# humeniuka/semiclassical

Measured on AMD Instinct MI355X. Metric: trajectory-steps/sec + wall-time to converged C(t), anharmonic-AS D=60, higher is better.
Workload: dtype f64

## Files before the change

### semiclassical_amd/csrc/sc_hk_lu.h

```cpp
#pragma once
#include "sc_common.h"

#ifdef LU_PIVOT_CLOCK
static __device__ unsigned long long *g_lu_clock = nullptr;
#endif

namespace {

template <int CTRL>
__device__ __forceinline__ int dpp_mov_i32(int v) {
    return __builtin_amdgcn_update_dpp(v, v, CTRL, 0xF, 0xF, false);
}

__device__ __forceinline__ int row16_max_i32(int v) {
    asm("s_nop 1\n\t"
        "v_max_i32_dpp %0, %0, %0 row_ror:8 row_mask:0xf bank_mask:0xf\n\ts_nop 1\n\t"
        "v_max_i32_dpp %0, %0, %0 row_ror:4 row_mask:0xf bank_mask:0xf\n\ts_nop 1\n\t"
        "v_max_i32_dpp %0, %0, %0 row_ror:2 row_mask:0xf bank_mask:0xf\n\ts_nop 1\n\t"
        "v_max_i32_dpp %0, %0, %0 row_ror:1 row_mask:0xf bank_mask:0xf"
        : "+v"(v));
    return v;
}

__device__ __forceinline__ double readlane_f64(double v, int src) {
    const int lo = __builtin_amdgcn_readlane(__double2loint(v), src);
    const int hi = __builtin_amdgcn_readlane(__double2hiint(v), src);
    return __hiloint2double(hi, lo);
}

__device__ __forceinline__ cplx c_inv_fast(cplx z) {
    const double x = c_abs2(z);
    double r = __builtin_amdgcn_rcp(x);
    r = fma(fma(-x, r, 1.0), r, r);
    r = fma(fma(-x, r, 1.0), r, r);
    return c_make(z.x * r, -z.y * r);
}

struct PivotRecord {
    int col, pad;
};

#define SC_DPP_MOV(o, i, P) "v_mov_b64_dpp %[" #o "], %[" #i "] row_newbcast:" #P " row_mask:0xf bank_mask:0xf\n\t"
#define SC_LEAF1(P) SC_DPP_MOV(ox0, ix0, P) SC_DPP_MOV(oy0, iy0, P) "s_branch .Lend_%=\n\t"
#define SC_LEAF2(P) SC_DPP_MOV(ox0, ix0, P) SC_DPP_MOV(oy0, iy0, P) SC_DPP_MOV(ox1, ix1, P) SC_DPP_MOV(oy1, iy1, P) \
    "s_branch .Lend_%=\n\t"
#define SC_LEAF3(P) SC_DPP_MOV(ox0, ix0, P) SC_DPP_MOV(oy0, iy0, P) SC_DPP_MOV(ox1, ix1, P) SC_DPP_MOV(oy1, iy1, P) \
    SC_DPP_MOV(ox2, ix2, P) SC_DPP_MOV(oy2, iy2, P) "s_branch .Lend_%=\n\t"
#define SC_LEAF4(P) SC_DPP_MOV(ox0, ix0, P) SC_DPP_MOV(oy0, iy0, P) SC_DPP_MOV(ox1, ix1, P) SC_DPP_MOV(oy1, iy1, P) \
    SC_DPP_MOV(ox2, ix2, P) SC_DPP_MOV(oy2, iy2, P) SC_DPP_MOV(ox3, ix3, P) SC_DPP_MOV(oy3, iy3, P) "s_branch .Lend_%=\n\t"
#define SC_LEAF5(P) SC_DPP_MOV(ox0, ix0, P) SC_DPP_MOV(oy0, iy0, P) SC_DPP_MOV(ox1, ix1, P) SC_DPP_MOV(oy1, iy1, P) \
    SC_DPP_MOV(ox2, ix2, P) SC_DPP_MOV(oy2, iy2, P) SC_DPP_MOV(ox3, ix3, P) SC_DPP_MOV(oy3, iy3, P)              \
    SC_DPP_MOV(ox4, ix4, P) SC_DPP_MOV(oy4, iy4, P) "s_branch .Lend_%=\n\t"
#define SC_LEAF6(P) SC_DPP_MOV(ox0, ix0, P) SC_DPP_MOV(oy0, iy0, P) SC_DPP_MOV(ox1, ix1, P) SC_DPP_MOV(oy1, iy1, P) \
    SC_DPP_MOV(ox2, ix2, P) SC_DPP_MOV(oy2, iy2, P) SC_DPP_MOV(ox3, ix3, P) SC_DPP_MOV(oy3, iy3, P)              \
    SC_DPP_MOV(ox4, ix4, P) SC_DPP_MOV(oy4, iy4, P) SC_DPP_MOV(ox5, ix5, P) SC_DPP_MOV(oy5, iy5, P) "s_branch .Lend_%=\n\t"
#define SC_LEAVES(L) L(0) L(1) L(2) L(3) L(4) L(5) L(6) L(7) L(8) L(9) L(10) L(11) L(12) L(13) L(14) L(15)
#define SC_JUMP(BYTES)                                                                           \
    "s_getpc_b64 vcc\n"                                                                          \
    ".Lbase_%=:\n\t"                                                                             \
    "s_mul_i32 %[t], %[pl], " #BYTES "\n\t"                                                      \
    "s_add_u32 vcc_lo, vcc_lo, %[t]\n\t"                                                         \
    "s_addc_u32 vcc_hi, vcc_hi, 0\n\t"                                                           \
    "s_add_u32 vcc_lo, vcc_lo, .Lleaf0_%=-.Lbase_%=\n\t"                                         \
    "s_addc_u32 vcc_hi, vcc_hi, 0\n\t"                                                           \
    "s_setpc_b64 vcc\n"                                                                          \
    ".Lleaf0_%=:\n\t"
#define SC_IN(n) [ix##n] "v"(m##n.x), [iy##n] "v"(m##n.y)
#define SC_OUT(n) [ox##n] "=&v"(c##n.x), [oy##n] "=&v"(c##n.y)

__device__ __forceinline__ void column_fetch_n(int pl, cplx m0, cplx &c0) {
    int t;
    asm volatile(SC_JUMP(20) SC_LEAVES(SC_LEAF1) ".Lend_%=:\n" : SC_OUT(0), [t] "=&s"(t) : SC_IN(0), [pl] "s"(pl) : "vcc", "scc");
}
__device__ __forceinline__ void column_fetch_n(int pl, cplx m0, cplx m1, cplx &c0, cplx &c1) {
    int t;
    asm volatile(SC_JUMP(36) SC_LEAVES(SC_LEAF2) ".Lend_%=:\n"
                 : SC_OUT(0), SC_OUT(1), [t] "=&s"(t) : SC_IN(0), SC_IN(1), [pl] "s"(pl) : "vcc", "scc");
}
__device__ __forceinline__ void column_fetch_n(int pl, cplx m0, cplx m1, cplx m2, cplx &c0, cplx &c1, cplx &c2) {
    int t;
    asm volatile(SC_JUMP(52) SC_LEAVES(SC_LEAF3) ".Lend_%=:\n"
                 : SC_OUT(0), SC_OUT(1), SC_OUT(2), [t] "=&s"(t) : SC_IN(0), SC_IN(1), SC_IN(2), [pl] "s"(pl) : "vcc", "scc");
}
__device__ __forceinline__ void column_fetch_n(int pl, cplx m0, cplx m1, cplx m2, cplx m3, cplx &c0, cplx &c1, cplx &c2,
                                               cplx &c3) {
    int t;
    asm volatile(SC_JUMP(68) SC_LEAVES(SC_LEAF4) ".Lend_%=:\n"
                 : SC_OUT(0), SC_OUT(1), SC_OUT(2), SC_OUT(3), [t] "=&s"(t)
                 : SC_IN(0), SC_IN(1), SC_IN(2), SC_IN(3), [pl] "s"(pl) : "vcc", "scc");
}

__device__ __forceinline__ void column_fetch_n(int pl, cplx m0, cplx m1, cplx m2, cplx m3, cplx m4, cplx &c0, cplx &c1, cplx &c2,
                                               cplx &c3, cplx &c4) {
    int t;
    asm volatile(SC_JUMP(84) SC_LEAVES(SC_LEAF5) ".Lend_%=:\n"
                 : SC_OUT(0), SC_OUT(1), SC_OUT(2), SC_OUT(3), SC_OUT(4), [t] "=&s"(t)
                 : SC_IN(0), SC_IN(1), SC_IN(2), SC_IN(3), SC_IN(4), [pl] "s"(pl) : "vcc", "scc");
}
__device__ __forceinline__ void column_fetch_n(int pl, cplx m0, cplx m1, cplx m2, cplx m3, cplx m4, cplx m5, cplx &c0, cplx &c1,
                                               cplx &c2, cplx &c3, cplx &c4, cplx &c5) {
    int t;
    asm volatile(SC_JUMP(100) SC_LEAVES(SC_LEAF6) ".Lend_%=:\n"
                 : SC_OUT(0), SC_OUT(1), SC_OUT(2), SC_OUT(3), SC_OUT(4), SC_OUT(5), [t] "=&s"(t)
                 : SC_IN(0), SC_IN(1), SC_IN(2), SC_IN(3), SC_IN(4), SC_IN(5), [pl] "s"(pl) : "vcc", "scc");
}

template <int NR, int KB>
__device__ __forceinline__ void column_fetch(const cplx (&m)[NR][NR], cplx (&c)[NR], int pl) {
    pl = __builtin_amdgcn_readfirstlane(pl);
    if constexpr (NR - KB == 1) column_fetch_n(pl, m[KB][KB], c[KB]);
    if constexpr (NR - KB == 2) column_fetch_n(pl, m[KB][KB], m[KB + 1][KB], c[KB], c[KB + 1]);
    if constexpr (NR - KB == 3) column_fetch_n(pl, m[KB][KB], m[KB + 1][KB], m[KB + 2][KB], c[KB], c[KB + 1], c[KB + 2]);
    if constexpr (NR - KB == 4)
        column_fetch_n(pl, m[KB][KB], m[KB + 1][KB], m[KB + 2][KB], m[KB + 3][KB], c[KB], c[KB + 1], c[KB + 2], c[KB + 3]);
    if constexpr (NR - KB == 5)
        column_fetch_n(pl, m[KB][KB], m[KB + 1][KB], m[KB + 2][KB], m[KB + 3][KB], m[KB + 4][KB], c[KB], c[KB + 1], c[KB + 2],
                       c[KB + 3], c[KB + 4]);
    if constexpr (NR - KB == 6)
        column_fetch_n(pl, m[KB][KB], m[KB + 1][KB], m[KB + 2][KB], m[KB + 3][KB], m[KB + 4][KB], m[KB + 5][KB], c[KB], c[KB + 1],
                       c[KB + 2], c[KB + 3], c[KB + 4], c[KB + 5]);
}

template <int NR, int KB, int RW>
__device__ __forceinline__ void publish_pivot_row(const cplx (&m)[NR][NR], cplx *detbuf, bool live, int kt, int seq,
                                                  cplx (*rowbuf)[RW], PivotRecord *pivrec, int *weak, int tid) {
    const int tj = tid & 15, lane = tid & 63;
    const int blk = (__double2hiint(c_abs2(m[KB][KB])) & ~15) | (15 - tj);
    int key_blk = live ? blk : -1;
    const cplx myinv = c_inv_fast(m[KB][KB]);
    key_blk = row16_max_i32(key_blk);
    const int pl = 15 - (key_blk & 15);
    const int src = __builtin_amdgcn_readfirstlane((lane & ~15) | pl);
    const cplx inv = c_make(readlane_f64(myinv.x, src), readlane_f64(myinv.y, src));
    rowbuf[kt][16 * KB + tj] = c_mul(m[KB][KB], inv);
#pragma unroll
    for (int rb = KB + 1; rb < NR; ++rb) rowbuf[kt][16 * rb + tj] = c_mul(m[KB][rb], inv);
    __asm__ volatile("" ::: "memory");
    if (tj == pl) {
        __hip_atomic_store(&pivrec[kt].pad, (seq << 4) | pl, __ATOMIC_RELAXED, __HIP_MEMORY_SCOPE_WORKGROUP);
#ifdef LU_PIVOT_CLOCK
        if (g_lu_clock && blockIdx.x == 0 && ((seq - 1 - KB) >> 2) < 64) g_lu_clock[(((seq - 1 - KB) >> 2) * 64 + 16 * KB + kt) * 4 + 2] = clock64();
#endif
    }
    __asm__ volatile("" ::: "memory");
    const unsigned long long lm = __ballot(live);
    const int flip = (__popcll(lm & ((1ull << src) - 1ull)) & 1) << 31;
    if (tj == pl) {
        const cplx piv = c_make(__hiloint2double(__double2hiint(m[KB][KB].x) ^ flip, __double2loint(m[KB][KB].x)),
                                __hiloint2double(__double2hiint(m[KB][KB].y) ^ flip, __double2loint(m[KB][KB].y)));
        detbuf[16 * KB + kt] = piv;
        if (m[KB][KB].x == 0.0 && m[KB][KB].y == 0.0) atomicOr(weak, 2);
    }
    __asm__ volatile("" ::: "memory");
    if (KB + 1 < NR) {
        int key_out = -1;
#pragma unroll
        for (int rb = KB + 1; rb < NR; ++rb) key_out = max(key_out, __double2hiint(c_abs2(m[KB][rb])));
        if ((key_out & ~15) - (key_blk & ~15) > (8 << 20)) atomicOr(weak, 1);
    }
}

__device__ __forceinline__ bool pivot_step_valid(int kt, int nk) { return 4 * (kt & 3) + (kt >> 2) < nk; }

#ifndef SC_LU_PEEL_LAST
#define SC_LU_PEEL_LAST 1
#endif
template <int NR, int KB>
__device__ __forceinline__ void column_fetch_below(const cplx (&m)[NR][NR], cplx (&c)[NR], int pl) {
    pl = __builtin_amdgcn_readfirstlane(pl);
    if constexpr (NR - KB == 2) column_fetch_n(pl, m[KB + 1][KB], c[KB + 1]);
    if constexpr (NR - KB == 3) column_fetch_n(pl, m[KB + 1][KB], m[KB + 2][KB], c[KB + 1], c[KB + 2]);
    if constexpr (NR - KB == 4) column_fetch_n(pl, m[KB + 1][KB], m[KB + 2][KB], m[KB + 3][KB], c[KB + 1], c[KB + 2], c[KB + 3]);
    if constexpr (NR - KB == 5)
        column_fetch_n(pl, m[KB + 1][KB], m[KB + 2][KB], m[KB + 3][KB], m[KB + 4][KB], c[KB + 1], c[KB + 2], c[KB + 3], c[KB + 4]);
    if constexpr (NR - KB == 6)
        column_fetch_n(pl, m[KB + 1][KB], m[KB + 2][KB], m[KB + 3][KB], m[KB + 4][KB], m[KB + 5][KB], c[KB + 1], c[KB + 2], c[KB + 3],
                       c[KB + 4], c[KB + 5]);
}

template <int NR, int KB, int RW, class Barrier>
__device__ __forceinline__ void eliminate_block(cplx (&m)[NR][NR], cplx *detbuf, int D, int seq,
                                                cplx (*rowbuf)[RW], PivotRecord *pivrec, int *weak, int tid,
                                                Barrier &&barrier) {
    const int ti = ((tid >> 4) & 3) * 4 + (tid >> 6), tj = tid & 15;
    constexpr bool FULL = KB + 1 < NR;
    const int nk = FULL ? 16 : min(16, D - 16 * KB);
    bool live = FULL ? true : 16 * KB + tj < D;
    barrier();
    if (ti == 0) publish_pivot_row<NR, KB, RW>(m, detbuf, live, 0, seq, rowbuf, pivrec, weak, tid);
    constexpr bool PEEL = SC_LU_PEEL_LAST != 0 && FULL;
    for (int kt = 0; kt < (PEEL ? 15 : 16); ++kt) {
        if (!FULL && !pivot_step_valid(kt, nk)) continue;
        int next = kt + 1;
        if (!FULL) while (next < 16 && !pivot_step_valid(next, nk)) ++next;
        int tag;
        cplx r[NR];
        for (;;) {
            tag = __builtin_amdgcn_readfirstlane(__hip_atomic_load(&pivrec[kt].pad, __ATOMIC_RELAXED, __HIP_MEMORY_SCOPE_WORKGROUP));
            __asm__ volatile("" ::: "memory");
#pragma unroll
            for (int rb = KB; rb < NR; ++rb) r[rb] = rowbuf[kt][16 * rb + tj];
            __asm__ volatile("" ::: "memory");
            if ((tag >> 4) == seq) break;
        }
        const int pl = tag & 15;
#ifdef LU_PIVOT_CLOCK
        if (g_lu_clock && blockIdx.x == 0 && next < 16 && ti == next && tj == 0 && ((seq - 1 - KB) >> 2) < 64)
            g_lu_clock[(((seq - 1 - KB) >> 2) * 64 + 16 * KB + next) * 4 + 0] = clock64();
#endif
        live = live && tj != pl;
        cplx c[NR];
        column_fetch<NR, KB>(m, c, pl);
#pragma unroll
        for (int rb = KB; rb < NR; ++rb) m[KB][rb] = c_fnma(c[KB], r[rb], m[KB][rb]);
#ifdef LU_PIVOT_CLOCK
        if (g_lu_clock && blockIdx.x == 0 && next < 16 && ti == next && tj == 0 && ((seq - 1 - KB) >> 2) < 64)
            g_lu_clock[(((seq - 1 - KB) >> 2) * 64 + 16 * KB + next) * 4 + 1] = clock64();
#endif
        if (next < 16 && ti == next) publish_pivot_row<NR, KB, RW>(m, detbuf, live, next, seq, rowbuf, pivrec, weak, tid);
#pragma unroll
        for (int ra = KB + 1; ra < NR; ++ra) {
#pragma unroll
            for (int rb = KB; rb < NR; ++rb) m[ra][rb] = c_fnma(c[ra], r[rb], m[ra][rb]);
        }
    }
    if constexpr (PEEL) {
        int tag;
        cplx r[NR];
        for (;;) {
            tag = __builtin_amdgcn_readfirstlane(__hip_atomic_load(&pivrec[15].pad, __ATOMIC_RELAXED, __HIP_MEMORY_SCOPE_WORKGROUP));
            __asm__ volatile("" ::: "memory");
#pragma unroll
            for (int rb = KB + 1; rb < NR; ++rb) r[rb] = rowbuf[15][16 * rb + tj];
            __asm__ volatile("" ::: "memory");
            if ((tag >> 4) == seq) break;
        }
        cplx c[NR];
        column_fetch_below<NR, KB>(m, c, tag & 15);
#pragma unroll
        for (int ra = KB + 1; ra < NR; ++ra) {
#pragma unroll
            for (int rb = KB + 1; rb < NR; ++rb) m[ra][rb] = c_fnma(c[ra], r[rb], m[ra][rb]);
        }
    }
}

template <int NR>
__device__ __forceinline__ void lu_partial_products(cplx *detbuf, int t) {
    cplx p = detbuf[t];
#pragma unroll
    for (int kb = 1; kb < NR; ++kb) p = c_mul(p, detbuf[16 * kb + t]);
    detbuf[t] = p;
    __builtin_amdgcn_fence(__ATOMIC_RELEASE, "wavefront");
}
__device__ __forceinline__ cplx finish_determinant(const cplx *detbuf, bool rows_odd) {
    __builtin_amdgcn_fence(__ATOMIC_ACQUIRE, "wavefront");
    cplx det = detbuf[0];
#pragma unroll
    for (int g = 1; g < 16; ++g) det = c_mul(det, detbuf[g]);
    return rows_odd ? c_make(-det.x, -det.y) : det;
}
__device__ __forceinline__ bool row_order_is_odd(int D) {
    int inversions = 0;
    for (int kb = 0; 16 * kb < D; ++kb) {
        const int nk = min(16, D - 16 * kb);
        for (int k1 = 0; k1 < 16; ++k1)
            for (int k2 = k1 + 1; k2 < 16; ++k2) {
                const int r1 = 4 * (k1 & 3) + (k1 >> 2), r2 = 4 * (k2 & 3) + (k2 >> 2);
                if (r1 < nk && r2 < nk && r1 > r2) ++inversions;
            }
    }
    return (inversions & 1) != 0;
}

}
```

### semiclassical_amd/csrc/sc_hk_step_sd.hip

```cpp
#include <algorithm>
#include "sc_common.h"
#include "sc_hk_lu.h"
#include "sc_row16.h"

#ifndef SC_SD_DEPTH
#define SC_SD_DEPTH 1
#endif
#ifndef SC_SD_XPREFETCH
#define SC_SD_XPREFETCH 1
#endif
#ifndef SC_SD_XPREFETCH2
#define SC_SD_XPREFETCH2 1
#endif
#ifndef SC_SD_XPREFETCH_AHEAD
#define SC_SD_XPREFETCH_AHEAD 1
#endif
#ifndef SC_SD_LOAD_AUX
#define SC_SD_LOAD_AUX 2
#endif
#ifndef SC_SD_MULTI_LOAD_AUX
#define SC_SD_MULTI_LOAD_AUX 2
#endif
#ifndef SC_SD_NOSTORE_LOAD_AUX
#define SC_SD_NOSTORE_LOAD_AUX 0
#endif
#ifndef SC_SD_MULTI_MID_AUX
#define SC_SD_MULTI_MID_AUX 0
#endif
#ifndef SC_SD_NOSTORE_MIN_NR
#define SC_SD_NOSTORE_MIN_NR 3
#endif
#ifndef SC_SD_STORE_AUX
#define SC_SD_STORE_AUX 2
#endif
#ifndef SC_SD_DIRECT_P
#define SC_SD_DIRECT_P 0
#endif
#ifndef SC_SD_ABLATE_LU
#define SC_SD_ABLATE_LU 0
#endif
#ifndef SC_SD_FORCE_FIXUP
#define SC_SD_FORCE_FIXUP 0
#endif
#ifndef SC_SD_BLOCK_BARRIER
#define SC_SD_BLOCK_BARRIER no_barrier
#endif

namespace {

typedef unsigned int sc_v2u __attribute__((ext_vector_type(2)));
typedef unsigned int sc_v4u __attribute__((ext_vector_type(4)));

struct MultiArgs {
    const double *work;
    double *c2_mid, *sgn_mid;
    int *unrepaired;
};

#ifdef SD_PHASE_CLOCK
__device__ unsigned long long *g_sd_clock = nullptr;
#define SD_TICK(i)                                                                                                       \
    do {                                                                                                                 \
        if (pc_blk >= 0 && pc_item < 256 && (threadIdx.x & 63) == 0)                                                     \
            g_sd_clock[((pc_blk * 4 + (threadIdx.x >> 6)) * 256 + pc_item) * 6 + (i)] = wall_clock64();                  \
    } while (0)
#else
#define SD_TICK(i) do { } while (0)
#endif

template <int NR, int MINW, bool STEP, bool TILED, int KS = 1>
__global__ __launch_bounds__(256, MINW) void hk_step_sd_kernel(StepArgs A, MultiArgs MA) {
#ifdef SD_PHASE_CLOCK
    const int pc_blk = g_sd_clock == nullptr ? -1 : (blockIdx.x == 0 ? 0 : (blockIdx.x == 512 ? 1 : -1));
    int pc_item = 0;
#endif
    constexpr bool mid_store = KS > 1 && NR < SC_SD_NOSTORE_MIN_NR;
    constexpr int NP = mid_store ? 1 : KS;
    constexpr bool late_p = KS >= 4 && NR >= 4;
    constexpr int aux_first = KS == 1 ? SC_SD_LOAD_AUX : (mid_store ? SC_SD_MULTI_LOAD_AUX : SC_SD_NOSTORE_LOAD_AUX);
    __shared__ double prop[NP][4 * 64];
    __shared__ double scl[4 * 64];
    __shared__ cplx rowbuf[16][64];
    __shared__ PivotRecord pivrec[16];
    __shared__ cplx detbuf[2][16 * NR];
    __shared__ int weakbuf[2];
    __shared__ int nextbuf[2];

    static_assert(KS == 1 || !SC_SD_DIRECT_P || NR < SC_SD_NOSTORE_MIN_NR, "a later sub-step of a visit needs the row propagators of the earlier ones (prop[])");
    const int D = A.st.dim, DD = D * D, tid = threadIdx.x;
    constexpr bool do_step = STEP;
    constexpr int NCL_BASE = 16 * (NR - 1);
    if (tid < 64) {
        const bool in = tid < D;
        const double st = in ? A.hk.st[tid] : 1.0, si = in ? A.hk.si[tid] : 1.0;
        if (tid < 16) pivrec[tid].pad = 0;
        if (tid < 2) { nextbuf[tid] = 0; weakbuf[tid] = 0; }
        scl[tid] = st; scl[64 + tid] = 1.0 / st; scl[128 + tid] = si; scl[192 + tid] = 1.0 / si;
#pragma unroll
        for (int k = 0; k < NP; ++k) { prop[k][tid] = 1.0; prop[k][64 + tid] = 0.0; prop[k][128 + tid] = 0.0; prop[k][192 + tid] = 1.0; }
    }
    __syncthreads();

    const bool rows_odd = row_order_is_odd(D);
    const int wave_s = __builtin_amdgcn_readfirstlane(tid >> 6);
    int seq0 = 0;
    int par = 0;
    double raw[2][4][NR];
    double pv[2][4] = {{1.0, 0.0, 0.0, 1.0}, {1.0, 0.0, 0.0, 1.0}};
    double prv = 0.0;
    bool first = true;
    int *cursor = A.st.flags ? A.st.flags + A.st.n + 1 : nullptr;
    int64_t trn = 0;
    for (int64_t tr = blockIdx.x; tr < A.st.n; tr = trn) {
      sfor<0, KS>([&](auto ksc) {
        constexpr int ks = decltype(ksc)::value;
        constexpr int aux_load = ks == 0 ? aux_first : SC_SD_MULTI_MID_AUX;
        constexpr int aux_store = ks == KS - 1 ? SC_SD_STORE_AUX : SC_SD_MULTI_MID_AUX;
        constexpr bool store_blocks = ks == KS - 1 || mid_store;
        constexpr int ksn = ks + 1 < KS ? ks + 1 : 0;
        int *weak = &weakbuf[par];
        unsigned ones = ~0u;
        __asm__ volatile("" : "+s"(ones));
        const int tl = (wave_s << 6) | (int)__builtin_amdgcn_mbcnt_hi(ones, __builtin_amdgcn_mbcnt_lo(ones, 0u));
        const int tj = tl & 15, tjl = tj;
        const int til = (tl >> 6) * 4 + ((tl >> 4) & 3);
        if (tl == 0) *weak = SC_SD_FORCE_FIXUP;
        if (tl < 16 * NR) {
            double one = 1.0, zero = 0.0;
            __asm__ volatile("" : "+v"(one), "+v"(zero));
            detbuf[par][tl] = c_make(one, zero);
        }
        int drawn = 0;
        if (ks == 0 && cursor && tl == 0) drawn = atomicAdd(cursor, 1);
        const int pk = tl >> 6, pa = tl & 63;

        cplx m[NR][NR];
        int Dl = D;
        __asm__ volatile("" : "+s"(Dl));
        constexpr unsigned OOB = 0x7fffffffu;
        const bool rowok_last = 16 * (NR - 1) + til < Dl, colok_last = NCL_BASE + tj < Dl;
        const unsigned vo = TILED ? 16u * (unsigned)(til * 16 + tj) : 8u * (unsigned)(til * Dl + tj);
        const unsigned vol = TILED ? 16u * (unsigned)(til * (Dl - NCL_BASE) + tj) : vo;
        auto voffset = [&](int ra, int rb) {
            const unsigned v = rb == NR - 1 ? vol : vo;
            const bool ok = (ra < NR - 1 || rowok_last) && (rb < NR - 1 || colok_last);
            return (int)((ra < NR - 1 && rb < NR - 1) ? v : (ok ? v : OOB));
        };
        auto tile_base = [&](int ra, int rb) {
            const int nra = min(16, Dl - 16 * ra);
            return 8 * (TILED ? 4 * (16 * ra * Dl + nra * 16 * rb) : 16 * ra * Dl + 16 * rb);
        };
        auto plane_bytes = [&](int ra, int rb) {
            const int nra = min(16, Dl - 16 * ra), ncb = rb == NR - 1 ? Dl - NCL_BASE : 16;
            return 8 * (TILED ? nra * ncb : Dl * Dl);
        };
        auto resource = [&](int64_t t) {
            return __builtin_amdgcn_make_buffer_rsrc(A.st.mono + t * 4 * (int64_t)Dl * Dl, 0, 32 * Dl * Dl, 0x00020000);
        };
        auto load_slot = [&](auto rac, int64_t t, auto auxc) {
            constexpr int ra = decltype(rac)::value, aux = decltype(auxc)::value;
            const __amdgpu_buffer_rsrc_t rs = resource(t);
#pragma unroll
            for (int rb = 0; rb < NR; ++rb) {
                const int vofs = voffset(ra, rb), base = tile_base(ra, rb), plane = plane_bytes(ra, rb);
                if constexpr (TILED) {
#pragma unroll
                    for (int pp = 0; pp < 2; ++pp) {
                        const sc_v4u v = __builtin_amdgcn_raw_buffer_load_b128(rs, vofs, base + pp * 2 * plane, aux);
                        raw[ra & 1][2 * pp][rb] = __hiloint2double((int)v.y, (int)v.x);
                        raw[ra & 1][2 * pp + 1][rb] = __hiloint2double((int)v.w, (int)v.z);
                    }
                } else {
#pragma unroll
                    for (int pl = 0; pl < 4; ++pl) {
                        const sc_v2u v = __builtin_amdgcn_raw_buffer_load_b64(rs, vofs, base + pl * plane, 0);
                        raw[ra & 1][pl][rb] = __hiloint2double((int)v.y, (int)v.x);
                    }
                }
            }
            if (SC_SD_DIRECT_P && do_step) {
                const __amdgpu_buffer_rsrc_t rw = __builtin_amdgcn_make_buffer_rsrc(A.st.work + t * 4 * (int64_t)Dl, 0, 32 * Dl, 0x00020000);
                const unsigned vw = 16 * ra + til < Dl ? 8u * (unsigned)(16 * ra + til) : OOB;
#pragma unroll
                for (int k = 0; k < 4; ++k) {
                    const sc_v2u v = __builtin_amdgcn_raw_buffer_load_b64(rw, (int)vw, 8 * k * Dl, 0);
                    pv[ra & 1][k] = __hiloint2double((int)v.y, (int)v.x);
                }
            }
        };
        auto first_requests = [&](int64_t t, auto ksnc) {
            constexpr int k2 = decltype(ksnc)::value;
            constexpr int aux2 = k2 == 0 ? aux_first : SC_SD_MULTI_MID_AUX;
            const double *wk = KS > 1 ? MA.work + (int64_t)k2 * A.st.n * 4 * Dl : A.st.work;
            if (!SC_SD_DIRECT_P && do_step && pa < Dl) prv = wk[(t * 4 + pk) * (int64_t)Dl + pa];
            load_slot(std::integral_constant<int, 0>(), t, std::integral_constant<int, aux2>());
            if (SC_SD_XPREFETCH2 && NR > 1) load_slot(std::integral_constant<int, (NR > 1 ? 1 : 0)>(), t, std::integral_constant<int, aux2>());
        };
        auto finish_slot = [&](auto rac) {
            constexpr int ra = decltype(rac)::value;
            const __amdgpu_buffer_rsrc_t rs = resource(tr);
            const int al = (16 * ra + til) & 63;
            if constexpr (ks > 0 && !mid_store) {
                sfor<0, ks>([&](auto kpc) {
                    constexpr int kp = decltype(kpc)::value;
                    WM_BLOCK {
                        const double q11 = prop[kp][al], q12 = prop[kp][64 + al], q21 = prop[kp][128 + al], q22 = prop[kp][192 + al];
#pragma unroll
                        for (int rb = 0; rb < NR; ++rb)
                            sep_propagate_row(q11, q12, q21, q22, raw[ra & 1][0][rb], raw[ra & 1][1][rb], raw[ra & 1][2][rb], raw[ra & 1][3][rb]);
                    }
                    __builtin_amdgcn_sched_barrier(0);
                });
            }
            constexpr int kq = mid_store ? 0 : ks;
            const double p11 = SC_SD_DIRECT_P ? pv[ra & 1][0] : prop[kq][al], p12 = SC_SD_DIRECT_P ? pv[ra & 1][1] : prop[kq][64 + al];
            const double p21 = SC_SD_DIRECT_P ? pv[ra & 1][2] : prop[kq][128 + al], p22 = SC_SD_DIRECT_P ? pv[ra & 1][3] : prop[kq][192 + al];
            const double sta = scl[al], ista = scl[64 + al];
#pragma unroll
            for (int rb = 0; rb < NR; ++rb) {
                const int vofs = voffset(ra, rb), base = tile_base(ra, rb), plane = plane_bytes(ra, rb);
                double mqq = raw[ra & 1][0][rb], mqp = raw[ra & 1][1][rb], mpq = raw[ra & 1][2][rb], mpp = raw[ra & 1][3][rb];
                if (do_step) {
                    sep_propagate_row(p11, p12, p21, p22, mqq, mqp, mpq, mpp);
                    const double out[4] = {mqq, mqp, mpq, mpp};
                    if constexpr (!store_blocks) {
                        (void)out; (void)rs; (void)vofs; (void)base; (void)plane;
                        __builtin_amdgcn_sched_barrier(0);
                    } else if constexpr (TILED) {
#pragma unroll
                        for (int pp = 0; pp < 2; ++pp) {
                            sc_v4u v;
                            v.x = (unsigned)__double2loint(out[2 * pp]); v.y = (unsigned)__double2hiint(out[2 * pp]);
                            v.z = (unsigned)__double2loint(out[2 * pp + 1]); v.w = (unsigned)__double2hiint(out[2 * pp + 1]);
                            __builtin_amdgcn_raw_buffer_store_b128(v, rs, vofs, base + pp * 2 * plane, aux_store);
                            __builtin_amdgcn_sched_barrier(0);
                            __asm__ volatile("s_nop 2");
                            __builtin_amdgcn_sched_barrier(0);
                        }
                    } else {
#pragma unroll
                        for (int pl = 0; pl < 4; ++pl) {
                            sc_v2u v;
                            v.x = (unsigned)__double2loint(out[pl]); v.y = (unsigned)__double2hiint(out[pl]);
                            __builtin_amdgcn_raw_buffer_store_b64(v, rs, vofs, base + pl * plane, 0);
                        }
                    }
                }
                const int bl = (16 * rb + tjl) & 63;
                const double sib = scl[128 + bl], isib = scl[192 + bl];
                m[ra][rb] = prefactor_element_diag(sta, ista, sib, isib, mqq, mqp, mpq, mpp);
                __asm__ volatile("" : "+v"(m[ra][rb].x), "+v"(m[ra][rb].y));
            }
        };
        SD_TICK(0);
        if constexpr (late_p) {
            if (!first && do_step && pa < Dl) prv = MA.work[(((int64_t)ks * A.st.n + tr) * 4 + pk) * (int64_t)Dl + pa];
        }
        if (first || !SC_SD_XPREFETCH || NR == 1) first_requests(tr, ksc);
        first = false;
        __builtin_amdgcn_sched_barrier(0);
        if (NR > 1 && SC_SD_DEPTH > 1) load_slot(std::integral_constant<int, (NR > 1 ? 1 : 0)>(), tr, std::integral_constant<int, aux_load>());
        __builtin_amdgcn_sched_barrier(0);
        if (do_step && !SC_SD_DIRECT_P) {
            if (pa < D) prop[mid_store ? 0 : ks][64 * pk + pa] = prv;
            __syncthreads();
        }
        sfor<0, NR>([&](auto rac) {
            constexpr int ra = decltype(rac)::value;
            if (SC_SD_DEPTH == 1 && ra > (SC_SD_XPREFETCH2 ? 1 : 0)) load_slot(rac, tr, std::integral_constant<int, aux_load>());
            if (SC_SD_DEPTH > 1 && ra + 1 < NR && ra > 0) load_slot(std::integral_constant<int, (ra + 1 < NR ? ra + 1 : 0)>(), tr, std::integral_constant<int, aux_load>());
            __builtin_amdgcn_sched_barrier(0);
            finish_slot(rac);
            __builtin_amdgcn_sched_barrier(0);
        });

        constexpr bool skip_lu = SC_SD_ABLATE_LU != 0;
        SD_TICK(1);
        if (ks == 0 && cursor && tl == 0) nextbuf[par] = drawn;
        __syncthreads();
        SD_TICK(2);
        auto wg_barrier = [] { __syncthreads(); };
        auto no_barrier = [] {};
        (void)no_barrier; (void)wg_barrier;
        sfor<0, NR>([&](auto kbc) {
            constexpr int KB = decltype(kbc)::value;
            if (ks == 0 && KB == (NR > 1 ? 1 : 0)) {
                if (NR > 1) trn = cursor ? (int64_t)gridDim.x + __builtin_amdgcn_readfirstlane(nextbuf[par]) : tr + gridDim.x;
            }
            if (SC_SD_XPREFETCH && NR > 1 && KB == (NR - SC_SD_XPREFETCH_AHEAD > 1 ? NR - SC_SD_XPREFETCH_AHEAD : 1)) {
                const int64_t tnext = ks + 1 < KS ? tr : trn;
                if (tnext < A.st.n) {
                    if constexpr (late_p) {
                        constexpr int auxn = ksn == 0 ? aux_first : SC_SD_MULTI_MID_AUX;
                        load_slot(std::integral_constant<int, 0>(), tnext, std::integral_constant<int, auxn>());
                        if (SC_SD_XPREFETCH2) load_slot(std::integral_constant<int, 1>(), tnext, std::integral_constant<int, auxn>());
                    } else {
                        first_requests(tnext, std::integral_constant<int, ksn>());
                    }
                } else {
                    prv = 0.0;
#pragma unroll
                    for (int pl = 0; pl < 4; ++pl) {
                        pv[0][pl] = 0.0;
#pragma unroll
                        for (int rb = 0; rb < NR; ++rb) {
                            raw[0][pl][rb] = 0.0;
                            if (SC_SD_XPREFETCH2) raw[1][pl][rb] = 0.0;
                        }
                    }
                }
            }
            if (!skip_lu) {
                if (KB == 0) eliminate_block<NR, KB, 64>(m, detbuf[par], D, seq0 + 1 + KB, rowbuf, pivrec, weak, tl, no_barrier);
                else eliminate_block<NR, KB, 64>(m, detbuf[par], D, seq0 + 1 + KB, rowbuf, pivrec, weak, tl, SC_SD_BLOCK_BARRIER);
            }
        });
        SD_TICK(3);
        __syncthreads();
        SD_TICK(4);
        if (ks == 0 && NR == 1) trn = cursor ? (int64_t)gridDim.x + __builtin_amdgcn_readfirstlane(nextbuf[par]) : tr + gridDim.x;
        cplx *c2 = (cplx *)A.st.c2;
        const cplx *c2_in = ks == 0 ? c2 + tr : (const cplx *)MA.c2_mid + ((int64_t)(ks - 1) * A.st.n + tr);
        const double *sg_in = ks == 0 ? A.st.sgn + tr : MA.sgn_mid + ((int64_t)(ks - 1) * A.st.n + tr);
        cplx *c2_out = ks == KS - 1 ? c2 + tr : (cplx *)MA.c2_mid + ((int64_t)ks * A.st.n + tr);
        double *sg_out = ks == KS - 1 ? A.st.sgn + tr : MA.sgn_mid + ((int64_t)ks * A.st.n + tr);
        if (tl < 16) lu_partial_products<NR>(detbuf[par], tl);
        if (ks == KS - 1 && tl == 0 && (*weak & 1) && A.st.flags && !skip_lu) {
            if (KS > 1) {
                c2[tr] = *c2_in;
                A.st.sgn[tr] = *sg_in;
            }
            A.st.flags[tr] = 1;
            atomicAdd(&A.st.flags[A.st.n], 1);
        } else if (tl == 0) {
            if (KS > 1 && ks < KS - 1 && (*weak & 1) && !skip_lu) atomicAdd(MA.unrepaired, 1);
            const cplx c2new = (*weak & 2) ? c_make(0.0, 0.0) : finish_determinant(detbuf[par], rows_odd);
            if (do_step) {
                const cplx prev = *c2_in;
                const double sg = *sg_in;
                const bool flip = crossed_branch_cut(prev, c2new);
                if (KS > 1) *sg_out = flip ? -sg : sg;
                else if (flip) *sg_out = -sg;
            } else {
                *sg_out = 1.0;
            }
            *c2_out = c2new;
        }
        seq0 += 4; par ^= 1;
        SD_TICK(5);
#ifdef SD_PHASE_CLOCK
        ++pc_item;
#endif
      });
    }
}

#ifdef SD_PHASE_CLOCK
}
extern "C" int sc_sd_phase_clock(unsigned long long *buf) {
    return hipMemcpyToSymbol(HIP_SYMBOL(g_sd_clock), &buf, sizeof(buf)) == hipSuccess ? 0 : -3;
}
namespace {
#endif

__global__ __launch_bounds__(256) void hk_modes_kernel(StepArgs A) {
    const int D = A.st.dim, lane = threadIdx.x & 63, wave = threadIdx.x >> 6;
    const double dt = A.dt, h6 = dt / 6.0;
    __shared__ double wsum[4];
    double esum = 0.0;
    for (int64_t tr = (int64_t)blockIdx.x * 4 + wave; tr < A.st.n; tr += (int64_t)gridDim.x * 4) {
        double *qp = A.st.qp + tr * 2 * D;
        double *pr = A.st.work + tr * 4 * (int64_t)D;
        double red5[5] = {0, 0, 0, 0, 0};
        if (lane < D) {
            const double im = A.pot.inv_mass[lane];
            const double c0 = A.pot.par0[lane], c1 = A.pot.par1 ? A.pot.par1[lane] : 0.0;
            double q = qp[lane], p = qp[D + lane], h1, h2, h3, h4, p11, p12, p21, p22;
            sep_mode_rk4(A.pot.kind, c0, c1, im, dt, q, p, red5, h1, h2, h3, h4);
            qp[lane] = q;
            qp[D + lane] = p;
            sep_row_propagator(im, h1, h2, h3, h4, dt, p11, p12, p21, p22);
            pr[lane] = p11; pr[D + lane] = p12; pr[2 * D + lane] = p21; pr[3 * D + lane] = p22;
        }
#pragma unroll
        for (int i = 0; i < 5; ++i) red5[i] = wave_sum(red5[i]);
        if (lane == 0) {
            A.st.act[tr] += h6 * (red5[0] + 2.0 * red5[1] + 2.0 * red5[2] + red5[3]);
            esum += red5[4];
        }
    }
    if (lane == 0) wsum[wave] = esum;
    __syncthreads();
    if (threadIdx.x == 0 && A.epart) A.epart[blockIdx.x] = wsum[0] + wsum[1] + wsum[2] + wsum[3];
}


struct ModesMultiArgs {
    double *work, *qp_mid, *act_mid;
};
template <int KS>
__global__ __launch_bounds__(256) void hk_modes_multi_kernel(StepArgs A, ModesMultiArgs MM) {
    const int D = A.st.dim, lane = threadIdx.x & 63, wave = threadIdx.x >> 6;
    const double dt = A.dt, h6 = dt / 6.0;
    __shared__ double wsum[KS][4];
    double esum[KS];
#pragma unroll
    for (int ks = 0; ks < KS; ++ks) esum[ks] = 0.0;
    for (int64_t tr = (int64_t)blockIdx.x * 4 + wave; tr < A.st.n; tr += (int64_t)gridDim.x * 4) {
        double *qp = A.st.qp + tr * 2 * D;
        const bool in = lane < D;
        double q = in ? qp[lane] : 0.0, p = in ? qp[D + lane] : 0.0;
        const double im = in ? A.pot.inv_mass[lane] : 0.0, c0 = in ? A.pot.par0[lane] : 0.0, c1 = (in && A.pot.par1) ? A.pot.par1[lane] : 0.0;
        double act = A.st.act[tr];
#pragma unroll
        for (int ks = 0; ks < KS; ++ks) {
            double *pr = MM.work + ((int64_t)ks * A.st.n + tr) * 4 * (int64_t)D;
            double red5[5] = {0, 0, 0, 0, 0};
            if (in) {
                double h1, h2, h3, h4, p11, p12, p21, p22;
                sep_mode_rk4(A.pot.kind, c0, c1, im, dt, q, p, red5, h1, h2, h3, h4);
                sep_row_propagator(im, h1, h2, h3, h4, dt, p11, p12, p21, p22);
                pr[lane] = p11; pr[D + lane] = p12; pr[2 * D + lane] = p21; pr[3 * D + lane] = p22;
                double *qo = ks == KS - 1 ? qp : MM.qp_mid + ((int64_t)ks * A.st.n + tr) * 2 * D;
                qo[lane] = q; qo[D + lane] = p;
            }
#pragma unroll
            for (int i = 0; i < 5; ++i) red5[i] = wave_sum(red5[i]);
            act += h6 * (red5[0] + 2.0 * red5[1] + 2.0 * red5[2] + red5[3]);
            if (lane == 0) {
                if (ks == KS - 1) A.st.act[tr] = act; else MM.act_mid[(int64_t)ks * A.st.n + tr] = act;
                esum[ks] += red5[4];
            }
        }
    }
#pragma unroll
    for (int ks = 0; ks < KS; ++ks) if (lane == 0) wsum[ks][wave] = esum[ks];
    __syncthreads();
    if (threadIdx.x < KS && A.epart)
        A.epart[(size_t)threadIdx.x * gridDim.x + blockIdx.x] = wsum[threadIdx.x][0] + wsum[threadIdx.x][1] + wsum[threadIdx.x][2] + wsum[threadIdx.x][3];
}

template <bool STEP>
__global__ __launch_bounds__(256) void hk_step_w16_kernel(StepArgs A) {
    __shared__ double prop[4][4][16];
    __shared__ double wsum[4];
    const int D = A.st.dim, DD = D * D, lane = threadIdx.x & 63, wave = threadIdx.x >> 6;
    const int rg = lane >> 4, tj = lane & 15;
    const double dt = A.dt, h6 = dt / 6.0;
    const bool colok = tj < D;
    const double sib = colok ? A.hk.si[tj] : 1.0, isib = 1.0 / sib;
    double sta[4], ista[4];
#pragma unroll
    for (int s = 0; s < 4; ++s) {
        const int r = rg + 4 * s;
        sta[s] = r < D ? A.hk.st[r] : 1.0;
        ista[s] = 1.0 / sta[s];
    }
    double esum = 0.0;
    for (int64_t tr = (int64_t)blockIdx.x * 4 + wave; tr < A.st.n; tr += (int64_t)gridDim.x * 4) {
        double *qp = A.st.qp + tr * 2 * D;
        double *M = A.st.mono + tr * 4 * (int64_t)DD;
        double p11[4] = {1, 1, 1, 1}, p12[4] = {0, 0, 0, 0}, p21[4] = {0, 0, 0, 0}, p22[4] = {1, 1, 1, 1};
        if (STEP) {
            double red5[5] = {0, 0, 0, 0, 0};
            if (lane < D) {
                const double im = A.pot.inv_mass[lane];
                const double c0 = A.pot.par0[lane], c1 = A.pot.par1 ? A.pot.par1[lane] : 0.0;
                double q = qp[lane], p = qp[D + lane], h1, h2, h3, h4, u1, u2, v1, v2;
                sep_mode_rk4(A.pot.kind, c0, c1, im, dt, q, p, red5, h1, h2, h3, h4);
                qp[lane] = q;
                qp[D + lane] = p;
                sep_row_propagator(im, h1, h2, h3, h4, dt, u1, u2, v1, v2);
                prop[wave][0][lane] = u1; prop[wave][1][lane] = u2; prop[wave][2][lane] = v1; prop[wave][3][lane] = v2;
            }
#pragma unroll
            for (int i = 0; i < 5; ++i) red5[i] = wave_sum(red5[i]);
            if (lane == 0) {
                A.st.act[tr] += h6 * (red5[0] + 2.0 * red5[1] + 2.0 * red5[2] + red5[3]);
                esum += red5[4];
            }
            __builtin_amdgcn_fence(__ATOMIC_RELEASE, "wavefront");
            __builtin_amdgcn_wave_barrier();
            __builtin_amdgcn_fence(__ATOMIC_ACQUIRE, "wavefront");
#pragma unroll
            for (int s = 0; s < 4; ++s) {
                const int r = rg + 4 * s;
                if (r < D) { p11[s] = prop[wave][0][r]; p12[s] = prop[wave][1][r]; p21[s] = prop[wave][2][r]; p22[s] = prop[wave][3][r]; }
            }
        }
        cplx m[4];
#pragma unroll
        for (int s = 0; s < 4; ++s) {
            const int r = rg + 4 * s;
            const bool ok = colok && r < D;
            const int e = r * D + tj;
            double mqq = ok ? M[e] : 0.0, mqp = ok ? M[DD + e] : 0.0, mpq = ok ? M[2 * DD + e] : 0.0, mpp = ok ? M[3 * DD + e] : 0.0;
            if (STEP) {
                sep_propagate_row(p11[s], p12[s], p21[s], p22[s], mqq, mqp, mpq, mpp);
                if (ok) { M[e] = mqq; M[DD + e] = mqp; M[2 * DD + e] = mpq; M[3 * DD + e] = mpp; }
            }
            m[s] = ok ? prefactor_element_diag(sta[s], ista[s], sib, isib, mqq, mqp, mpq, mpp) : c_make(r == tj ? 1.0 : 0.0, 0.0);
        }
        cplx det = c_make(1.0, 0.0);
        bool live = colok, singular = false;
        int parity = 0;
#pragma unroll
        for (int k = 0; k < 16; ++k) {
            if (k < D && !singular) {
                constexpr int dummy = 0; (void)dummy;
                const int rgk = k & 3, sk = k >> 2;
                const int blk = (__double2hiint(c_abs2(m[sk])) & ~15) | (15 - tj);
                const int keymax = row16_max_i32((live && rg == rgk) ? blk : -1);
                const int kb = __builtin_amdgcn_readlane(keymax, 16 * rgk);
                const int pl = 15 - (kb & 15);
                const int src = 16 * rgk + pl;
                const cplx piv = c_make(readlane_f64(m[sk].x, src), readlane_f64(m[sk].y, src));
                if (piv.x == 0.0 && piv.y == 0.0) { singular = true; }
                else {
                    det = c_mul(det, piv);
                    const cplx inv = c_inv_fast(piv);
                    const unsigned long long lm = __ballot(live && rg == 0);
                    parity ^= __popcll(lm & ((1ull << pl) - 1ull)) & 1;
                    const cplx rowv = c_make(__shfl(m[sk].x, 16 * rgk + tj, 64), __shfl(m[sk].y, 16 * rgk + tj, 64));
                    const bool keep = live && tj != pl;
                    const cplx rs = c_mul(rowv, inv);
                    const cplx r = c_make(keep ? rs.x : 0.0, keep ? rs.y : 0.0);
                    cplx c[4];
                    column_fetch_n(pl, m[0], m[1], m[2], m[3], c[0], c[1], c[2], c[3]);
#pragma unroll
                    for (int s = 0; s < 4; ++s) {
                        if (rg + 4 * s <= k) c[s] = c_make(0.0, 0.0);
                        m[s] = c_fnma(c[s], r, m[s]);
                    }
                    live = live && tj != pl;
                }
            }
        }
        if (lane == 0) {
            if (singular) det = c_make(0.0, 0.0);
            else if (parity) det = c_make(-det.x, -det.y);
            cplx *c2 = (cplx *)A.st.c2;
            if (STEP) {
                const cplx prev = c2[tr];
                if (crossed_branch_cut(prev, det)) A.st.sgn[tr] = -A.st.sgn[tr];
            } else {
                A.st.sgn[tr] = 1.0;
            }
            c2[tr] = det;
        }
    }
    if (lane == 0) wsum[wave] = esum;
    __syncthreads();
    if (threadIdx.x == 0 && A.epart && STEP) A.epart[blockIdx.x] = wsum[0] + wsum[1] + wsum[2] + wsum[3];
}

}

#ifdef SC_TUNING
int sc_launch_step_ws(const StepArgs &a, hipStream_t s);
#endif

int sc_launch_step_sd(const StepArgs &a, hipStream_t s) {
    const int D = a.st.dim, nr = (D + 15) / 16, grid = sc_step_grid(a.st.n, D);
    int occ = 4;
    bool wave_kernel = D <= 16;
#ifdef SC_TUNING
    if (const char *occ_env = getenv("SC_SD_OCC")) occ = atoi(occ_env);
    if (getenv("SC_NO_WAVE_KERNEL")) wave_kernel = false;
#endif
    if (wave_kernel) {
        bool packed = true;
#ifdef SC_TUNING
        if (getenv("SC_NO_SEP16")) packed = false;
#endif
        if (packed) {
            const int rc = sc_launch_step_sep16(a, grid, s);
            if (rc != 0) return rc < 0 ? rc : SC_OK;
        }
        const int64_t quads = (a.st.n + 3) / 4;
        const int wg = (int)(quads < 2048 ? quads : 2048);
        if (a.epart && hipMemsetAsync(a.epart, 0, sizeof(double) * (size_t)grid, s) != hipSuccess)
            return sc_check_launch("sc_hk_step (partials)");
        if ((a.mode & 0xff) == 0) hipLaunchKernelGGL(hk_step_w16_kernel<true>, dim3(wg), dim3(256), 0, s, a);
        else hipLaunchKernelGGL(hk_step_w16_kernel<false>, dim3(wg), dim3(256), 0, s, a);
        return sc_check_launch("sc_hk_step (one wavefront per trajectory)");
    }
    if ((a.mode & 0xff) == 0) hipLaunchKernelGGL(hk_modes_kernel, dim3(grid), dim3(256), 0, s, a);
    const bool step = (a.mode & 0xff) == 0;
    const bool tiled = a.st.mono_layout == SC_MONO_TILED16;
#ifdef SC_TUNING
    if (nr == 4 && step && a.mode == 0 && getenv("SC_WS")) return sc_launch_step_ws(a, s);
#endif
    int sdgrid = grid;
#ifdef SC_TUNING
    if (const char *g = getenv("SC_SD_GRID")) sdgrid = (int)std::min<int64_t>(a.st.n, atoi(g));
#endif
#define SC_LAUNCH_SD(NR_, OCC_)                                                                                         \
    do {                                                                                                                \
        if (step && tiled) hipLaunchKernelGGL((hk_step_sd_kernel<NR_, OCC_, true, true>), dim3(sdgrid), dim3(256), 0, s, a, MultiArgs{});   \
        else if (step) hipLaunchKernelGGL((hk_step_sd_kernel<NR_, OCC_, true, false>), dim3(sdgrid), dim3(256), 0, s, a, MultiArgs{});     \
        else if (tiled) hipLaunchKernelGGL((hk_step_sd_kernel<NR_, OCC_, false, true>), dim3(sdgrid), dim3(256), 0, s, a, MultiArgs{});    \
        else hipLaunchKernelGGL((hk_step_sd_kernel<NR_, OCC_, false, false>), dim3(sdgrid), dim3(256), 0, s, a, MultiArgs{});              \
    } while (0)
    switch (nr) {
        case 1: SC_LAUNCH_SD(1, 4); break;
        case 2: SC_LAUNCH_SD(2, 4); break;
        case 3: SC_LAUNCH_SD(3, 4); break;
        default:
#ifdef SC_TUNING
            if (occ == 3) { SC_LAUNCH_SD(4, 3); break; }
            if (occ < 3) { SC_LAUNCH_SD(4, 2); break; }
#endif
            (void)occ;
            SC_LAUNCH_SD(4, 4);
            break;
    }
#undef SC_LAUNCH_SD
    return sc_check_launch("sc_hk_step (separable/diagonal fast path)");
}

template <int KS>
static int launch_step_sd_visit(const StepArgs &a, const sc_multi_scratch &ms, hipStream_t s) {
    const int D = a.st.dim, nr = (D + 15) / 16, grid = sc_step_grid(a.st.n, D);
    ModesMultiArgs mm{ms.work, ms.qp_mid, ms.act_mid};
    hipLaunchKernelGGL(hk_modes_multi_kernel<KS>, dim3(grid), dim3(256), 0, s, a, mm);
    int rc = sc_check_launch("sc_hk_step_visit (modes)");
    if (rc) return rc;
    MultiArgs ma{ms.work, ms.c2_mid, ms.sgn_mid, ms.unrepaired};
    switch (nr) {
        case 3: hipLaunchKernelGGL((hk_step_sd_kernel<3, 4, true, true, KS>), dim3(grid), dim3(256), 0, s, a, ma); break;
        case 4: hipLaunchKernelGGL((hk_step_sd_kernel<4, 4, true, true, KS>), dim3(grid), dim3(256), 0, s, a, ma); break;
        default: return sc_fail(SC_ERR_UNSUPPORTED, "sc_hk_step_visit: %d steps per visit at D = %d", KS, D);
    }
    return sc_check_launch("sc_hk_step_visit (KS steps per visit)");
}

int sc_launch_step_sd_multi(const StepArgs &a, const sc_multi_scratch &ms, int ksteps, hipStream_t s) {
    if (ksteps == 3) return launch_step_sd_visit<3>(a, ms, s);
    if (ksteps == 4) return launch_step_sd_visit<4>(a, ms, s);
    if (ksteps != 2) return sc_fail(SC_ERR_UNSUPPORTED, "sc_hk_step_visit: %d steps per visit", ksteps);
    const int D = a.st.dim, nr = (D + 15) / 16, grid = sc_step_grid(a.st.n, D);
    ModesMultiArgs mm{ms.work, ms.qp_mid, ms.act_mid};
    hipLaunchKernelGGL(hk_modes_multi_kernel<2>, dim3(grid), dim3(256), 0, s, a, mm);
    int rc = sc_check_launch("sc_hk_step_multi (modes)");
    if (rc) return rc;
    MultiArgs ma{ms.work, ms.c2_mid, ms.sgn_mid, ms.unrepaired};
    switch (nr) {
        case 2: hipLaunchKernelGGL((hk_step_sd_kernel<2, 4, true, true, 2>), dim3(grid), dim3(256), 0, s, a, ma); break;
        case 3: hipLaunchKernelGGL((hk_step_sd_kernel<3, 4, true, true, 2>), dim3(grid), dim3(256), 0, s, a, ma); break;
        case 4:
#ifdef SC_TUNING
            if (const char *occ_env = getenv("SC_SD_OCC")) {
                if (atoi(occ_env) == 3) { hipLaunchKernelGGL((hk_step_sd_kernel<4, 3, true, true, 2>), dim3(grid), dim3(256), 0, s, a, ma); break; }
                if (atoi(occ_env) == 2) { hipLaunchKernelGGL((hk_step_sd_kernel<4, 2, true, true, 2>), dim3(grid), dim3(256), 0, s, a, ma); break; }
            }
#endif
            hipLaunchKernelGGL((hk_step_sd_kernel<4, 4, true, true, 2>), dim3(grid), dim3(256), 0, s, a, ma); break;
        default: return sc_fail(SC_ERR_UNSUPPORTED, "sc_hk_step_multi: D = %d", D);
    }
    return sc_check_launch("sc_hk_step_multi (two steps per visit)");
}

#ifdef LU_PIVOT_CLOCK
extern "C" int sc_lu_pivot_clock(unsigned long long *buf) {
    return hipMemcpyToSymbol(HIP_SYMBOL(g_lu_clock), &buf, sizeof(buf)) == hipSuccess ? 0 : -3;
}
#endif
```

Measured before the change: 29.25 million.

## Defer determinant tail into next item's load phase and trim last LU block

```diff
diff --git a/semiclassical_amd/csrc/sc_hk_lu.h b/semiclassical_amd/csrc/sc_hk_lu.h
--- a/semiclassical_amd/csrc/sc_hk_lu.h
+++ b/semiclassical_amd/csrc/sc_hk_lu.h
@@ -178,7 +178,7 @@
                        c[KB + 4], c[KB + 5]);
 }
 
-template <int NR, int KB, int RW, class Barrier>
+template <int NR, int KB, int RW, bool TRIM_LAST = false, class Barrier>
 __device__ __forceinline__ void eliminate_block(cplx (&m)[NR][NR], cplx *detbuf, int D, int seq,
                                                 cplx (*rowbuf)[RW], PivotRecord *pivrec, int *weak, int tid,
                                                 Barrier &&barrier) {
@@ -189,7 +189,13 @@
     barrier();
     if (ti == 0) publish_pivot_row<NR, KB, RW>(m, detbuf, live, 0, seq, rowbuf, pivrec, weak, tid);
     constexpr bool PEEL = SC_LU_PEEL_LAST != 0 && FULL;
-    for (int kt = 0; kt < (PEEL ? 15 : 16); ++kt) {
+    int kend = PEEL ? 15 : 16;
+    if constexpr (TRIM_LAST && !FULL) {
+        const int w = __builtin_amdgcn_readfirstlane(tid >> 6);
+        const int jl = min(3, nk - 1 - 4 * w);
+        kend = jl < 0 ? 0 : 4 * jl + w;
+    }
+    for (int kt = 0; kt < kend; ++kt) {
         if (!FULL && !pivot_step_valid(kt, nk)) continue;
         int next = kt + 1;
         if (!FULL) while (next < 16 && !pivot_step_valid(next, nk)) ++next;
diff --git a/semiclassical_amd/csrc/sc_hk_step_sd.hip b/semiclassical_amd/csrc/sc_hk_step_sd.hip
--- a/semiclassical_amd/csrc/sc_hk_step_sd.hip
+++ b/semiclassical_amd/csrc/sc_hk_step_sd.hip
@@ -41,6 +41,12 @@
 #endif
 #ifndef SC_SD_FORCE_FIXUP
 #define SC_SD_FORCE_FIXUP 0
+#endif
+#ifndef SC_SD_DEFER_TAIL
+#define SC_SD_DEFER_TAIL 1
+#endif
+#ifndef SC_SD_TRIM_LAST
+#define SC_SD_TRIM_LAST 1
 #endif
 #ifndef SC_SD_BLOCK_BARRIER
 #define SC_SD_BLOCK_BARRIER no_barrier
@@ -85,6 +91,8 @@
     __shared__ cplx detbuf[2][16 * NR];
     __shared__ int weakbuf[2];
     __shared__ int nextbuf[2];
+    __shared__ double tailkeep[4];
+    __shared__ long long tailtr;
 
     static_assert(KS == 1 || !SC_SD_DIRECT_P || NR < SC_SD_NOSTORE_MIN_NR, "a later sub-step of a visit needs the row propagators of the earlier ones (prop[])");
     const int D = A.st.dim, DD = D * D, tid = threadIdx.x;
@@ -111,6 +119,50 @@
     bool first = true;
     int *cursor = A.st.flags ? A.st.flags + A.st.n + 1 : nullptr;
     int64_t trn = 0;
+    constexpr bool defer_tail = SC_SD_DEFER_TAIL != 0;
+    constexpr bool skip_lu = SC_SD_ABLATE_LU != 0;
+    auto item_tail = [&](auto kpc, int64_t tp, int parp, int tl) {
+        constexpr int kp = decltype(kpc)::value;
+        if (tl >= 16) return;
+        if (tp < 0) tp = tailtr;
+        cplx *c2 = (cplx *)A.st.c2;
+        const cplx *c2_in = kp == 0 ? c2 + tp : (const cplx *)MA.c2_mid + ((int64_t)(kp - 1) * A.st.n + tp);
+        const double *sg_in = kp == 0 ? A.st.sgn + tp : MA.sgn_mid + ((int64_t)(kp - 1) * A.st.n + tp);
+        cplx *c2_out = kp == KS - 1 ? c2 + tp : (cplx *)MA.c2_mid + ((int64_t)kp * A.st.n + tp);
+        double *sg_out = kp == KS - 1 ? A.st.sgn + tp : MA.sgn_mid + ((int64_t)kp * A.st.n + tp);
+        const int *weak = &weakbuf[parp];
+        constexpr bool kept = defer_tail && kp > 0;
+        cplx prev = c_make(0.0, 0.0);
+        double sg = 1.0;
+        if (defer_tail && tl == 0 && do_step) {
+            if (kept) { prev = c_make(tailkeep[0], tailkeep[1]); sg = tailkeep[2]; }
+            else { prev = *c2_in; sg = *sg_in; }
+        }
+        if (tl < 16) lu_partial_products<NR>(detbuf[parp], tl);
+        if (kp == KS - 1 && tl == 0 && (*weak & 1) && A.st.flags && !skip_lu) {
+            if (KS > 1) {
+                c2[tp] = defer_tail ? prev : *c2_in;
+                A.st.sgn[tp] = defer_tail ? sg : *sg_in;
+            }
+            A.st.flags[tp] = 1;
+            atomicAdd(&A.st.flags[A.st.n], 1);
+        } else if (tl == 0) {
+            if (KS > 1 && kp < KS - 1 && (*weak & 1) && !skip_lu) atomicAdd(MA.unrepaired, 1);
+            const cplx c2new = (*weak & 2) ? c_make(0.0, 0.0) : finish_determinant(detbuf[parp], rows_odd);
+            double sgnew = 1.0;
+            if (do_step) {
+                if (!defer_tail) { prev = *c2_in; sg = *sg_in; }
+                const bool flip = crossed_branch_cut(prev, c2new);
+                sgnew = flip ? -sg : sg;
+                if (KS > 1) *sg_out = sgnew;
+                else if (flip) *sg_out = sgnew;
+            } else {
+                *sg_out = 1.0;
+            }
+            *c2_out = c2new;
+            if (defer_tail && kp < KS - 1) { tailkeep[0] = c2new.x; tailkeep[1] = c2new.y; tailkeep[2] = sgnew; }
+        }
+    };
     for (int64_t tr = blockIdx.x; tr < A.st.n; tr = trn) {
       sfor<0, KS>([&](auto ksc) {
         constexpr int ks = decltype(ksc)::value;
@@ -257,6 +309,7 @@
             if (!first && do_step && pa < Dl) prv = MA.work[(((int64_t)ks * A.st.n + tr) * 4 + pk) * (int64_t)Dl + pa];
         }
         if (first || !SC_SD_XPREFETCH || NR == 1) first_requests(tr, ksc);
+        const bool had_item = !first;
         first = false;
         __builtin_amdgcn_sched_barrier(0);
         if (NR > 1 && SC_SD_DEPTH > 1) load_slot(std::integral_constant<int, (NR > 1 ? 1 : 0)>(), tr, std::integral_constant<int, aux_load>());
@@ -270,11 +323,15 @@
             if (SC_SD_DEPTH == 1 && ra > (SC_SD_XPREFETCH2 ? 1 : 0)) load_slot(rac, tr, std::integral_constant<int, aux_load>());
             if (SC_SD_DEPTH > 1 && ra + 1 < NR && ra > 0) load_slot(std::integral_constant<int, (ra + 1 < NR ? ra + 1 : 0)>(), tr, std::integral_constant<int, aux_load>());
             __builtin_amdgcn_sched_barrier(0);
+            if constexpr (defer_tail && ra == (NR < 3 ? NR - 1 : 2)) {
+                if constexpr (ks > 0) item_tail(std::integral_constant<int, ks - 1>(), tr, par ^ 1, tl);
+                else if (had_item) item_tail(std::integral_constant<int, KS - 1>(), -1, par ^ 1, tl);
+                __builtin_amdgcn_sched_barrier(0);
+            }
             finish_slot(rac);
             __builtin_amdgcn_sched_barrier(0);
         });
 
-        constexpr bool skip_lu = SC_SD_ABLATE_LU != 0;
         SD_TICK(1);
         if (ks == 0 && cursor && tl == 0) nextbuf[par] = drawn;
         __syncthreads();
@@ -311,41 +368,17 @@
                 }
             }
             if (!skip_lu) {
-                if (KB == 0) eliminate_block<NR, KB, 64>(m, detbuf[par], D, seq0 + 1 + KB, rowbuf, pivrec, weak, tl, no_barrier);
-                else eliminate_block<NR, KB, 64>(m, detbuf[par], D, seq0 + 1 + KB, rowbuf, pivrec, weak, tl, SC_SD_BLOCK_BARRIER);
+                constexpr bool trim = SC_SD_TRIM_LAST != 0;
+                if (KB == 0) eliminate_block<NR, KB, 64, trim>(m, detbuf[par], D, seq0 + 1 + KB, rowbuf, pivrec, weak, tl, no_barrier);
+                else eliminate_block<NR, KB, 64, trim>(m, detbuf[par], D, seq0 + 1 + KB, rowbuf, pivrec, weak, tl, SC_SD_BLOCK_BARRIER);
             }
         });
         SD_TICK(3);
         __syncthreads();
         SD_TICK(4);
         if (ks == 0 && NR == 1) trn = cursor ? (int64_t)gridDim.x + __builtin_amdgcn_readfirstlane(nextbuf[par]) : tr + gridDim.x;
-        cplx *c2 = (cplx *)A.st.c2;
-        const cplx *c2_in = ks == 0 ? c2 + tr : (const cplx *)MA.c2_mid + ((int64_t)(ks - 1) * A.st.n + tr);
-        const double *sg_in = ks == 0 ? A.st.sgn + tr : MA.sgn_mid + ((int64_t)(ks - 1) * A.st.n + tr);
-        cplx *c2_out = ks == KS - 1 ? c2 + tr : (cplx *)MA.c2_mid + ((int64_t)ks * A.st.n + tr);
-        double *sg_out = ks == KS - 1 ? A.st.sgn + tr : MA.sgn_mid + ((int64_t)ks * A.st.n + tr);
-        if (tl < 16) lu_partial_products<NR>(detbuf[par], tl);
-        if (ks == KS - 1 && tl == 0 && (*weak & 1) && A.st.flags && !skip_lu) {
-            if (KS > 1) {
-                c2[tr] = *c2_in;
-                A.st.sgn[tr] = *sg_in;
-            }
-            A.st.flags[tr] = 1;
-            atomicAdd(&A.st.flags[A.st.n], 1);
-        } else if (tl == 0) {
-            if (KS > 1 && ks < KS - 1 && (*weak & 1) && !skip_lu) atomicAdd(MA.unrepaired, 1);
-            const cplx c2new = (*weak & 2) ? c_make(0.0, 0.0) : finish_determinant(detbuf[par], rows_odd);
-            if (do_step) {
-                const cplx prev = *c2_in;
-                const double sg = *sg_in;
-                const bool flip = crossed_branch_cut(prev, c2new);
-                if (KS > 1) *sg_out = flip ? -sg : sg;
-                else if (flip) *sg_out = -sg;
-            } else {
-                *sg_out = 1.0;
-            }
-            *c2_out = c2new;
-        }
+        if constexpr (defer_tail) { if (ks == KS - 1 && tl == 0) tailtr = tr; }
+        else item_tail(ksc, tr, par, tl);
         seq0 += 4; par ^= 1;
         SD_TICK(5);
 #ifdef SD_PHASE_CLOCK
@@ -353,6 +386,7 @@
 #endif
       });
     }
+    if (defer_tail && !first) item_tail(std::integral_constant<int, KS - 1>(), -1, par ^ 1, tid);
 }
 
 #ifdef SD_PHASE_CLOCK
```

New measurement: 29.89 million, median of 6. 1.02x the previous value.
